# CoderWZW/ARLib

Measured on AMD Instinct MI355X. Metric: BPR-train interactions/sec (LightGCN d=64 L=3 + BPR + Adam, B=2048), higher is better.
Workload: dtype f32

## Files before the change

arlib_amd/_lib.py:

```python
import ctypes as C
import os

_HERE = os.path.dirname(os.path.abspath(__file__))
LIB_PATH = os.environ.get('ARLIB_AMD_LIB') or os.path.join(_HERE, 'lib', 'libarlib_amd.so')
ABI_VERSION = 34
_lib = None


class ArlError(RuntimeError):
    pass


class arl_csr(C.Structure):
    _fields_ = [('n_rows', C.c_int64), ('nnz', C.c_int64), ('rowptr', C.c_void_p), ('col', C.c_void_p), ('val', C.c_void_p),
                ('chunk', C.c_int32), ('n_chunks', C.c_int64), ('chunk_row', C.c_void_p), ('chunk_begin', C.c_void_p),
                ('chunk_end', C.c_void_p), ('n_long', C.c_int64), ('long_row', C.c_void_p), ('long_first', C.c_void_p),
                ('long_count', C.c_void_p), ('partial', C.c_void_p), ('row_tasks', C.c_void_p)]


class arl_blocked(C.Structure):
    _fields_ = [('n_waves', C.c_int64), ('rows_per_wave', C.c_int64), ('loads_in_flight', C.c_int64), ('wave_ptr', C.c_void_p), ('wave_rows', C.c_void_p), ('rec_col', C.c_void_p),
                ('rec_val', C.c_void_p), ('n_split', C.c_int64), ('split_row', C.c_void_p), ('split_first', C.c_void_p), ('split_count', C.c_void_p),
                ('partial', C.c_void_p), ('waves_per_group', C.c_int64)]

# ... 17 lines not shown
    'arl_spmm_blocked_flagged_f32': (C.c_int, [C.POINTER(arl_blocked), _vp, _i64, _vp, _f, _f, _vp, _vp, _vp, _vp]),
    'arl_spmm_csr_rscale_f32': (C.c_int, [C.POINTER(arl_csr), _vp, _i64, _vp, _f, _f, _vp, _vp, _vp]),
    'arl_spmm_blocked_rscale_f32': (C.c_int, [C.POINTER(arl_blocked), _vp, _i64, _vp, _f, _f, _vp, _vp, _vp]),
    'arl_spmm_blocked_layersum_f32': (C.c_int, [C.POINTER(arl_blocked), _vp, _i64, _vp, _vp, _vp, _vp]),
    'arl_spmm_blocked_adam_f32': (C.c_int, [C.POINTER(arl_blocked), _vp, _i64, _f, _f, _vp, _vp, _vp, _vp, _vp, _f, _f, _f, _f, _i64, _vp]),
    'arl_lpt_deal': (C.c_int, [_i64, _vp, _i64, _i64, _vp, _vp]),
    'arl_syn_v1_pairs': (_i64, [_i64, _i64, C.c_double, C.c_uint64, C.c_double, _i64, _i64, _vp, _i64]),
    'arl_graph_digest': (C.c_uint64, [_vp, _i64]),
    'arl_spmm_csr_flagged_f32': (C.c_int, [C.POINTER(arl_csr), _vp, _i64, _vp, _f, _f, _vp, _vp, _vp, _vp]),
    'arl_spmm_csr_rows_workspace_bytes': (_i64, [_i64, _i64, _i64]),
    'arl_spmm_csr_rows_f32': (C.c_int, [C.POINTER(arl_csr), _vp, _i64, _vp, _i64, _i64, _vp, _i64, _f, _vp, _vp, _vp, _vp]),
    'arl_spmm_csr_rows_pieces_f32': (C.c_int, [C.POINTER(arl_csr), _vp, _i64, _vp, _i64, _i64, _i64, _vp, _i64, _f, _vp, _vp, _vp, _vp]),
    'arl_spmm_csr_rows_scratch_offset': (_i64, [_i64, _i64, _i64]),
    'arl_mark_rows_u8': (C.c_int, [_vp, _vp, _i64, _i32, _vp]),
    'arl_mark_rows_bits_u32': (C.c_int, [_vp, _vp, _i64, _i32, _vp]),
    'arl_zero_rows_f32': (C.c_int, [_vp, _vp, _i64, _i64, _vp]),
    'arl_batch_rows_set_f32': (C.c_int, [_vp, _vp, _vp, _vp, _i64, _i64, _vp, _f, _vp, _vp, _vp]),
    'arl_batch_rows_clear_f32': (C.c_int, [_vp, _vp, _vp, _vp, _i64, _i64, _vp, _vp]),
    'arl_bpr_l2_workspace_bytes': (_i64, [_i64]),
    'arl_bpr_l2_fwd_bwd_f32': (C.c_int, [_vp, _i64, _i64, _vp, _vp, _vp, _i64, _f, _f, _vp, _vp, _vp, _i32, _vp]),
    'arl_bpr_l2_partial_f32': (C.c_int, [_vp, _i64, _i64, _vp, _vp, _vp, _i64, _i64, _vp, _vp, _vp]),
    'arl_bpr_l2_backward_f32': (C.c_int, [_vp, _i64, _i64, _vp, _vp, _vp, _i64, _f, _f, _vp, _vp, _vp, _vp]),
    'arl_adam_dense_f32': (C.c_int, [_vp, _vp, _vp, _vp, _i64, _f, _f, _f, _f, _i64, _vp]),
    'arl_sgd_dense_f32': (C.c_int, [_vp, _vp, _i64, _f, _vp]),
    'arl_gather_rows_f32': (C.c_int, [_vp, _vp, _i64, _i64, _vp, _vp]),
    'arl_scatter_add_rows_f32': (C.c_int, [_vp, _vp, _i64, _i64, _vp, _f, _vp]),
    'arl_rows_axpy_unique_f32': (C.c_int, [_vp, _vp, _vp, _i64, _i64, _f, _vp, _vp]),
    'arl_shard_batch_prep_i32': (C.c_int, [_vp, _vp, _vp, _i64, _i64, _i64, _vp, _vp, _vp, _vp, _vp]),
    'arl_infonce_workspace_bytes': (_i64, [_i64, _i64]),
    'arl_infonce_fwd_bwd_f32': (C.c_int, [_vp, _vp, _i64, _i64, _f, _f, _vp, _vp, _vp, _vp, _vp]),
    'arl_simgcl_perturb_f32': (C.c_int, [_vp, _vp, _i64, _i64, _f, _vp]),
    'arl_simgcl_perturb_rng_f32': (C.c_int, [_vp, _vp, _i64, _i64, _vp, _f, C.c_uint64, C.c_uint64, _vp]),
    'arl_ngcf_combine_f32': (C.c_int, [_vp, _vp, _i64, _i64, _vp, _vp]),
    'arl_ngcf_act_f32': (C.c_int, [_vp, _vp, _i64, _i64, _f, _vp]),
    'arl_ngcf_act_bwd_f32': (C.c_int, [_vp, _vp, _i64, _i64, _f, _vp, _vp]),
    'arl_ngcf_combine_bwd_f32': (C.c_int, [_vp, _vp, _vp, _i64, _i64, _vp, _vp, _vp]),
    'arl_ngcf_dense_fwd_f32': (C.c_int, [_vp, _vp, _vp, _i64, _i64, _f, _vp, _vp]),
    'arl_ngcf_dense_dgrad_f32': (C.c_int, [_vp, _vp, _vp, _vp, _vp, _i64, _i64, _f, _vp, _vp, _vp, _vp]),
    'arl_ngcf_wgrad_workspace_bytes': (_i64, [_i64, _i64]),
    'arl_ngcf_dense_wgrad_f32': (C.c_int, [_vp, _vp, _vp, _i64, _i64, _vp, _vp, _vp]),
    'arl_ncf_tower_fwd_f32': (C.c_int, [_vp, _vp, _vp, _i64, _i64, _vp, _vp, _vp, _vp, _vp, _vp, _vp, _vp, _vp, _vp]),
    'arl_ncf_tower_bwd_workspace_bytes': (_i64, [_i64, _i64]),
    'arl_ncf_tower_bwd_f32': (C.c_int, [_vp, _vp, _vp, _vp, _vp, _vp, _i64, _i64, _vp, _vp, _vp, _vp, _vp, _vp, _vp]),
    'arl_wrmf_l2_workspace_bytes': (_i64, [_i64]),
    'arl_wrmf_l2_fwd_bwd_f32': (C.c_int, [_vp, _i64, _i64, _vp, _vp, _vp, _i64, _f, _f, _f, _vp, _vp, _vp, _i32, _vp]),
    'arl_bpr_adv_workspace_bytes': (_i64, [_i64, _i64]),
    'arl_bpr_adv_fwd_bwd_f32': (C.c_int, [_vp, _i64, _i64, _vp, _vp, _vp, _i64, _vp, _f, _f, _vp, _vp, _vp, _vp, _i32, _vp]),
    'arl_sfa_workspace_bytes': (_i64, [_i64, _i64]),
    'arl_sfa_l1_fwd_bwd_f32': (C.c_int, [_vp, _vp, _vp, _i64, _i64, _i64, _f, C.c_int32, _vp, _vp, _vp, _vp]),
    'arl_sfa_stage1_f32': (C.c_int, [_vp, _vp, _vp, _i64, _i64, _vp, _vp, _vp]),
# ... 105 lines not shown
```

arlib_amd/csrc/arl_kernels.hip:

```cpp
#include <hip/hip_runtime.h>
#include <stdint.h>
#include <math.h>
#include <stdio.h>
#include "arlib_amd.h"
#include "arl_ordered.h"
#include <type_traits>

#define ARL_LAUNCH_CHECK()                                  \
    do {                                                    \
        hipError_t e__ = hipGetLastError();                 \
        if (e__ != hipSuccess) return (int)e__;             \
    } while (0)

namespace {

constexpr int kWave = 64;
constexpr int kBlock = 256;
constexpr int kWavesPerBlock = kBlock / kWave;

__device__ __forceinline__ float wave_sum(float v) {
#pragma unroll
    for (int off = 32; off > 0; off >>= 1) v += __shfl_xor(v, off);
    return v;
}
// ... 957 lines not shown
}

__global__ __launch_bounds__(kBlock) void rows_axpy_unique_kernel(float *__restrict__ dst, const float *__restrict__ src, const int32_t *__restrict__ idx,
                                                                   int c0, int c1, int d, float alpha, const uint32_t *__restrict__ dup, int lds_n) {
    extern __shared__ int32_t srows[];
    const int lane = threadIdx.x & 63;
    const int t = c0 + blockIdx.x * kWavesPerBlock + (threadIdx.x >> 6);
    const bool valid = t < c1;
    const long long row = valid ? idx[t] : 0;
    const bool scan = valid && (!dup || ((dup[row >> 5] >> (row & 31)) & 1u));
    if (lds_n > 0) {
        if (__syncthreads_or(scan)) stage_rows(srows, 0, lds_n, [&](int j) { return idx[j]; });
        if (!valid) return;
        if (scan && !ordered_scan_lds(srows, 0, t, t, (int)row, lane, [&](int) {})) return;
    } else {
        if (!valid) return;
        if (scan && !ordered_scan(0, t, t, row, lane, [&](int j) { return idx[j]; }, [&](int) {})) return;
    }
    float *o = dst + (size_t)row * d;
    const float *x = src + (size_t)row * d;
    for (int k = lane; k < d; k += kWave) o[k] = fmaf(alpha, x[k], o[k]);
}

__global__ __launch_bounds__(kBlock) void shard_batch_prep_kernel(const int32_t *__restrict__ u, const int32_t *__restrict__ p, const int32_t *__restrict__ n,
                                                                   int B, int u0, int u1, int32_t *__restrict__ lu, float *__restrict__ own,
                                                                   int32_t *__restrict__ item_rows, int32_t *__restrict__ rows_l) {
    const int b = blockIdx.x * kBlock + threadIdx.x;
    if (b >= B) return;
    const int Ul = u1 - u0;
    const int uu = u[b];
    const int l = min(max(uu - u0, 0), max(Ul - 1, 0));
    lu[b] = l; own[b] = (uu >= u0 && uu < u1) ? 1.f : 0.f; own[B + b] = 1.f; own[2 * B + b] = 1.f;
    const int pp = p[b], nn = n[b];
    item_rows[b] = pp; item_rows[B + b] = nn;
    rows_l[b] = l; rows_l[B + b] = Ul + pp; rows_l[2 * B + b] = Ul + nn;
}

__global__ __launch_bounds__(kBlock) void bpr_bwd_kernel(const float *__restrict__ emb, int d, long long item_off,
                                                          const int32_t *__restrict__ ui, const int32_t *__restrict__ pi,
                                                          const int32_t *__restrict__ ni, int B, float reg, float upstream,
                                                          const float *__restrict__ ws, const float *__restrict__ out,
                                                          float *__restrict__ G, int c0, int c1, int distinct) {
    extern __shared__ int32_t srows[];
    const int lane = threadIdx.x & 63;
    const int t = c0 + blockIdx.x * kWavesPerBlock + (threadIdx.x >> 6);
#define ARL_ROWOF_BPR(j) ((j) < B ? (long long)ui[j] : ((j) < 2 * B ? item_off + pi[(j) - B] : item_off + ni[(j) - 2 * B]))
    if (!distinct) stage_rows(srows, c0, c1, [&](int j) { return ARL_ROWOF_BPR(j); });
    if (t >= c1) return;
    const int row = (int)ARL_ROWOF_BPR(t);
    const float cu = out[2] > 0.f ? upstream * reg / out[2] : 0.f, cp = out[3] > 0.f ? upstream * reg / out[3] : 0.f;
    float *o = G + (size_t)row * d;
    const float *own = emb + (size_t)row * d;
    for (int k0 = 0; k0 < d; k0 += 256) {
        float acc[4], mine[4];
#pragma unroll
        for (int i = 0; i < 4; ++i) { const int k = k0 + 64 * i + lane; acc[i] = k < d ? o[k] : 0.f; mine[i] = k < d ? own[k] : 0.f; }
        auto term = [&](int tt) {
            const int kind = tt / B, b = tt - kind * B;
            const float g = ws[b] * upstream;
            const float *x = emb + (size_t)(kind == 0 ? item_off + pi[b] : (long long)ui[b]) * d;
            const float *y = emb + (size_t)(item_off + ni[b]) * d;
#pragma unroll
            for (int i = 0; i < 4; ++i) {
                const int k = k0 + 64 * i + lane;
                if (k < d) {
                    float c;
                    if (kind == 0) c = fmaf(g, x[k] - y[k], cu * mine[i]);
                    else if (kind == 1) c = fmaf(g, x[k], cp * mine[i]);
                    else c = -g * x[k];
                    acc[i] = __fadd_rn(acc[i], c);
                }
            }
        };
        if (distinct) term(t);
        else if (!ordered_scan_lds(srows, c0, c1, t, row, lane, term)) return;
#pragma unroll
        for (int i = 0; i < 4; ++i) { const int k = k0 + 64 * i + lane; if (k < d) o[k] = acc[i]; }
    }
#undef ARL_ROWOF_BPR
}

__global__ __launch_bounds__(kBlock) void adam_kernel(float4 *__restrict__ p, const float4 *__restrict__ g, float4 *__restrict__ m,
                                                       float4 *__restrict__ v, long long n4, float step_size, float bc2_sqrt,
                                                       float w1, float b2, float w2, float eps) {
    for (long long i = (long long)blockIdx.x * kBlock + threadIdx.x; i < n4; i += (long long)gridDim.x * kBlock) {
        const float4 g4 = g[i];
        float4 p4 = p[i], m4 = m[i], v4 = v[i];
        float gg[4] = {g4.x, g4.y, g4.z, g4.w}, pp[4] = {p4.x, p4.y, p4.z, p4.w}, mm[4] = {m4.x, m4.y, m4.z, m4.w}, vv[4] = {v4.x, v4.y, v4.z, v4.w};
#pragma unroll
        for (int k = 0; k < 4; ++k) {
            mm[k] = mm[k] + (gg[k] - mm[k]) * w1;
            vv[k] = vv[k] * b2 + w2 * gg[k] * gg[k];
            pp[k] = pp[k] - step_size * (mm[k] / (sqrtf(vv[k]) / bc2_sqrt + eps));
        }
        p[i] = make_float4(pp[0], pp[1], pp[2], pp[3]); m[i] = make_float4(mm[0], mm[1], mm[2], mm[3]); v[i] = make_float4(vv[0], vv[1], vv[2], vv[3]);
    }
}
__global__ __launch_bounds__(kBlock) void adam_scalar_kernel(float *p, const float *g, float *m, float *v, long long from, long long n,
                                                              float step_size, float bc2_sqrt, float w1, float b2, float w2, float eps) {
    for (long long i = from + (long long)blockIdx.x * kBlock + threadIdx.x; i < n; i += (long long)gridDim.x * kBlock) {
        const float gi = g[i];
        const float mi = m[i] + (gi - m[i]) * w1;
        const float vi = v[i] * b2 + w2 * gi * gi;
        m[i] = mi; v[i] = vi;
        p[i] = p[i] - step_size * (mi / (sqrtf(vi) / bc2_sqrt + eps));
    }
}
__global__ __launch_bounds__(kBlock) void sgd_kernel(float *__restrict__ p, const float *__restrict__ g, long long n, float lr) {
    for (long long i = (long long)blockIdx.x * kBlock + threadIdx.x; i < n; i += (long long)gridDim.x * kBlock) p[i] = p[i] - lr * g[i];
}

// ... 2931 lines not shown
    if (!dst || !idx) return ARL_E_NULL;
    if (n < 0 || d <= 0 || n > 0x7fffffffll || d > 0x7fffffffll) return ARL_E_ARG;
    if (n == 0) return ARL_OK;
    hipLaunchKernelGGL(zero_rows_kernel, dim3((unsigned)((n + kWavesPerBlock - 1) / kWavesPerBlock)), dim3(kBlock), 0, (hipStream_t)stream, dst, idx, (int)n, (int)d);
    ARL_LAUNCH_CHECK();
    return ARL_OK;
}

int64_t arl_bpr_l2_workspace_bytes(int64_t B) { return B < 0 ? 0 : (int64_t)sizeof(float) * 4 * B; }

int arl_bpr_l2_fwd_bwd_f32(const float *emb, int64_t d, int64_t item_off, const int32_t *u, const int32_t *p, const int32_t *n, int64_t B,
                           float reg, float upstream, float *loss_out, float *G, void *workspace, int32_t distinct_rows, arl_stream_t stream) {
    if (!emb || !u || !p || !n || !loss_out || !workspace) return ARL_E_NULL;
    if (d <= 0 || B <= 0 || item_off < 0) return ARL_E_ARG;
    if (B > 0x7fffffffll / 4 || d > 0x7fffffffll) return ARL_E_RANGE;
    hipStream_t st = (hipStream_t)stream;
    float *ws = (float *)workspace;
    const unsigned grid = (unsigned)((B + kWavesPerBlock - 1) / kWavesPerBlock);
    hipLaunchKernelGGL(bpr_fwd_kernel, dim3(grid), dim3(kBlock), 0, st, emb, (int)d, (long long)item_off, u, p, n, (int)B, (float)B, ws);
    ARL_LAUNCH_CHECK();
    hipLaunchKernelGGL(bpr_finalize_kernel, dim3(1), dim3(kBlock), 0, st, (int)B, reg, ws, loss_out, 0);
    ARL_LAUNCH_CHECK();
    if (G) {
        const int rc = launch_bpr_bwd(emb, d, item_off, u, p, n, B, reg, upstream, ws, loss_out, G, st, distinct_rows != 0);
        if (rc) return rc;
    }
    return ARL_OK;
}

int arl_bpr_l2_partial_f32(const float *emb, int64_t d, int64_t item_off, const int32_t *u, const int32_t *p, const int32_t *n, int64_t B_local,
                           int64_t B_global, float *sums_out, void *workspace, arl_stream_t stream) {
    if (!emb || !sums_out || !workspace) return ARL_E_NULL;
    if (B_local > 0 && (!u || !p || !n)) return ARL_E_NULL;
    if (d <= 0 || B_local < 0 || B_global < B_local || B_global <= 0 || item_off < 0) return ARL_E_ARG;
    if (B_local > 0x7fffffffll / 4 || d > 0x7fffffffll) return ARL_E_RANGE;
    hipStream_t st = (hipStream_t)stream;
    float *ws = (float *)workspace;
    if (B_local > 0) {
        const unsigned grid = (unsigned)((B_local + kWavesPerBlock - 1) / kWavesPerBlock);
        hipLaunchKernelGGL(bpr_fwd_kernel, dim3(grid), dim3(kBlock), 0, st, emb, (int)d, (long long)item_off, u, p, n, (int)B_local, (float)B_global, ws);
        ARL_LAUNCH_CHECK();
    }
    hipLaunchKernelGGL(bpr_finalize_kernel, dim3(1), dim3(kBlock), 0, st, (int)B_local, 0.f, ws, sums_out, 1);
    ARL_LAUNCH_CHECK();
    return ARL_OK;
}

int arl_bpr_l2_backward_f32(const float *emb, int64_t d, int64_t item_off, const int32_t *u, const int32_t *p, const int32_t *n, int64_t B_local,
                            float reg, float upstream, const float *norms4, float *G, const void *workspace, arl_stream_t stream) {
    if (!emb || !norms4 || !G || !workspace) return ARL_E_NULL;
    if (B_local > 0 && (!u || !p || !n)) return ARL_E_NULL;
    if (d <= 0 || B_local < 0 || item_off < 0) return ARL_E_ARG;
    if (B_local > 0x7fffffffll / 4 || d > 0x7fffffffll) return ARL_E_RANGE;
    if (B_local == 0) return ARL_OK;
    return launch_bpr_bwd(emb, d, item_off, u, p, n, B_local, reg, upstream, (const float *)workspace, norms4, G, (hipStream_t)stream);
}

int arl_adam_dense_f32(float *p, const float *g, float *m, float *v, int64_t n, float lr, float beta1, float beta2, float eps, int64_t step,
                       arl_stream_t stream) {
    if (!p || !g || !m || !v) return ARL_E_NULL;
    if (n < 0 || step < 1) return ARL_E_ARG;
    if (n == 0) return ARL_OK;
    const AdamScalars a = adam_scalars(lr, beta1, beta2, step);
    hipStream_t st = (hipStream_t)stream;
    const bool al = (((uintptr_t)p | (uintptr_t)g | (uintptr_t)m | (uintptr_t)v) & 15u) == 0;
    const long long n4 = al ? n / 4 : 0;
    if (n4 > 0) {
        hipLaunchKernelGGL(adam_kernel, dim3(grid_for(n4, kBlock)), dim3(kBlock), 0, st, (float4 *)p, (const float4 *)g, (float4 *)m, (float4 *)v, n4,
                           a.step_size, a.bc2_sqrt, a.w1, a.b2, a.w2, eps);
        ARL_LAUNCH_CHECK();
    }
    if (n4 * 4 < n) {
        hipLaunchKernelGGL(adam_scalar_kernel, dim3(grid_for(n - n4 * 4, kBlock)), dim3(kBlock), 0, st, p, g, m, v, n4 * 4, (long long)n, a.step_size,
                           a.bc2_sqrt, a.w1, a.b2, a.w2, eps);
        ARL_LAUNCH_CHECK();
    }
    return ARL_OK;
}

int arl_sgd_dense_f32(float *p, const float *g, int64_t n, float lr, arl_stream_t stream) {
    if (!p || !g) return ARL_E_NULL;
    if (n < 0) return ARL_E_ARG;
    if (n == 0) return ARL_OK;
    hipLaunchKernelGGL(sgd_kernel, dim3(grid_for(n, kBlock)), dim3(kBlock), 0, (hipStream_t)stream, p, g, (long long)n, lr);
    ARL_LAUNCH_CHECK();
    return ARL_OK;
}

int arl_tables_sum_f32(const float *const *tables, int64_t n_tables, int64_t n_elems, float alpha, float *out, arl_stream_t stream) {
    if (!tables || !out) return ARL_E_NULL;
    if (n_tables < 1 || n_tables > 8 || n_elems < 0 || (n_elems & 3)) return ARL_E_ARG;
    if (n_elems == 0) return ARL_OK;
// ... 21 lines not shown
    if (n < 0 || d <= 0 || n > 0x7fffffffll || d > 0x7fffffffll) return ARL_E_ARG;
    if (n == 0) return ARL_OK;
    for (int64_t c0 = 0; c0 < n; c0 += kOrderedWindow) {
        const int64_t c1 = c0 + kOrderedWindow < n ? c0 + kOrderedWindow : n;
        hipLaunchKernelGGL(rows_add_ordered_kernel<false>, dim3((unsigned)((c1 - c0 + kWavesPerBlock - 1) / kWavesPerBlock)), dim3(kBlock), (size_t)(c1 - c0) * 4,
                           (hipStream_t)stream, dst, (uint8_t *)nullptr, (uint32_t *)nullptr, idx, (int)c0, (int)c1, (int)d, src, scale, (const float *)nullptr,
                           (const uint32_t *)nullptr);
        ARL_LAUNCH_CHECK();
    }
    return ARL_OK;
}

int arl_rows_axpy_unique_f32(float *dst, const float *src, const int32_t *idx, int64_t n, int64_t d, float alpha, const uint32_t *dup_bits,
                             arl_stream_t stream) {
    if (!src || !idx || !dst) return ARL_E_NULL;
    if (n < 0 || d <= 0 || n > 0x7fffffffll || d > 0x7fffffffll || dst == src) return ARL_E_ARG;
    for (int64_t c0 = 0; c0 < n; c0 += kOrderedWindow) {
        const int64_t c1 = c0 + kOrderedWindow < n ? c0 + kOrderedWindow : n;
        const int lds_n = n <= kOrderedWindow ? (int)n : 0;
        hipLaunchKernelGGL(rows_axpy_unique_kernel, dim3((unsigned)((c1 - c0 + kWavesPerBlock - 1) / kWavesPerBlock)), dim3(kBlock), (size_t)lds_n * 4,
                           (hipStream_t)stream, dst, src, idx, (int)c0, (int)c1, (int)d, alpha, dup_bits, lds_n);
        ARL_LAUNCH_CHECK();
    }
    return ARL_OK;
}

int arl_shard_batch_prep_i32(const int32_t *u, const int32_t *p, const int32_t *n, int64_t B, int64_t u0, int64_t u1, int32_t *lu, float *own,
                             int32_t *item_rows, int32_t *rows_l, arl_stream_t stream) {
    if (!u || !p || !n || !lu || !own || !item_rows || !rows_l) return ARL_E_NULL;
    if (B < 0 || B > 0x7fffffffll / 3 || u0 < 0 || u1 < u0 || u1 > 0x7fffffffll) return ARL_E_ARG;
    if (B == 0) return ARL_OK;
    hipLaunchKernelGGL(shard_batch_prep_kernel, dim3((unsigned)((B + kBlock - 1) / kBlock)), dim3(kBlock), 0, (hipStream_t)stream, u, p, n, (int)B, (int)u0,
                       (int)u1, lu, own, item_rows, rows_l);
    ARL_LAUNCH_CHECK();
    return ARL_OK;
}

static int nce_allrows_splits(int64_t nA, int64_t nV) {
    const int64_t row_blocks = (nA + 63) / 64;
    int64_t s = (2048 + row_blocks - 1) / row_blocks;
    const int64_t max_s = (nV + 4095) / 4096;
    if (s > max_s) s = max_s;
    if (s > 512) s = 512;
    return (int)(s < 1 ? 1 : s);
}

// ... 855 lines not shown
```

arlib_amd/dist_engine.py:

```python
import ctypes as C
import os
from functools import partial

import numpy as np
import torch

from .attack._common import cw_term


class _TimedWork:

    def __init__(self, work, comm):
        self.work, self.comm = work, comm

    def wait(self):
        c = self.comm
        e0 = torch.cuda.Event(enable_timing=True); e1 = torch.cuda.Event(enable_timing=True)
        e0.record()
        self.work.wait()
        e1.record()
        c.waits.append((e0, e1))
        return True


# ... 378 lines not shown
        for h in range(L - 1):
            src, dst = layers[-1], self.hops[h]
            k.spmm(self.Ai, src, out=dst[Ul:])
            if pending is not None:
                pending.wait()
            pending = self.comm.all_reduce_async(dst[Ul:])
            k.spmm(self.Au, src, out=dst[:Ul])
            layers.append(dst)
        X = layers[-1]
        if pending is not None and L >= 2:
            mine = [t[Ul:] for j, t in enumerate(layers[:-1]) if j % self.world == self.rank]
        else:
            mine = [t[Ul:] for j, t in enumerate(layers) if j % self.world == self.rank]
        k.spmm_rows(self.Ai, X, item_rows, mine, s, out=self.C[B:], check_range=False)
        if pending is not None:
            pending.wait()
            if L >= 2 and (L - 1) % self.world == self.rank:
                self.C[B:].add_(k.gather_rows(X, item_rows_packed, check_range=False), alpha=s)
        if Ul:
            k.spmm_rows(self.Au, X, lu, [t[:Ul] for t in layers], s, out=self.C[:B], check_range=False, row_weight=own[:B])
        else:
            self.C[:B].zero_()
        self.comm.all_reduce(self.C)
        self.Gc.zero_()
        k.bpr_l2_fwd_bwd(self.C, B, self.ar, self.ar, self.arB, self.reg, self.Gc, workspace=self.ws, loss_out=self.loss_out, check_range=False, distinct_rows=True)
        k.batch_rows_set_(self.G, self.flags, self.bits, rows_l, self.Gc, 1.0, check_range=False, row_scale=own, dup_bits=self.dup_bits)
        self.t += 1
        zu = self.flags[:Ul]
        acc = self.G
        pending, prev_items, prev_a = None, None, 1.0
        for h in range(L):
            last = h == L - 1
            a = s if last else 1.0
            dst = self.hops[h % len(self.hops)]
            if dst is acc:
                dst = self.hops[(h + 1) % len(self.hops)]
            xf = self.bits if h == 0 else None
            k.spmm_flagged(self.Ai, acc, xf, a, 0.0, None, None, out=dst[Ul:])
            if pending is not None:
                pending.wait()
                k.rows_axpy_unique_(prev_items, self.G, item_rows_packed, prev_a, check_range=False, dup_bits=self.dup_bits)
            pending, prev_items, prev_a = self.comm.all_reduce_async(dst[Ul:]), dst, a
            if last:
                k.spmm_adam(self.Au, acc, a, a, self.G[:Ul], self.E0[:Ul], self.m[:Ul], self.v[:Ul], self.lr, self.t, self.betas, self.eps, zflags=zu)
            else:
                k.spmm_flagged(self.Au, acc, xf, a, a, self.G[:Ul], zu, out=dst[:Ul])
            acc = dst
        pending.wait()
        k.rows_axpy_unique_(prev_items, self.G, item_rows_packed, prev_a, check_range=False, dup_bits=self.dup_bits)
        k.adam_dense(self.E0[Ul:], acc[Ul:], self.m[Ul:], self.v[Ul:], self.lr, self.t, self.betas, self.eps)
        k.batch_rows_clear_(self.G, self.flags, self.bits, rows_l, check_range=False, dup_bits=self.dup_bits)
        return self.loss_out

    def step_simgcl(self, u, p, n, cl_rate=0.2, tau=0.2, eps=0.1, noises=None):
        if not self.skip0:
            raise ValueError('step_simgcl needs skip_layer0=True (SimGCL averages layers 1..L)')
        k, L, Ul, d, dev = self.k, self.L, self.Ul, self.d, self.device
        if self.S1 is None:
            self.S1, self.S2 = torch.zeros_like(self.S), torch.zeros_like(self.S)

        def noise(view, hop):
            if noises is not None:
                return noises[view][hop]
            g = torch.Generator(device=dev)
            g.manual_seed(0x51AC1 + 7919 * self.t + 2 * hop + view)
            item = torch.rand(self.I, d, generator=g, device=dev)
            return torch.cat([torch.rand(Ul, d, device=dev), item], 0)

        def perturb(view, h, dst):
            if noises is None and hasattr(k, 'simgcl_perturb_rng'):
                if self._gid is None:
                    self._gid = torch.cat([torch.arange(self.u0, self.u1, device=dev), torch.arange(self.U, self.U + self.I, device=dev)]).to(torch.int32)
                k.simgcl_perturb_rng(dst, eps, 0x51AC1, (self.t * 2 + view) * L + h, out=dst, row_ids=self._gid)
# ... 164 lines not shown
```

arlib_amd/engine.py:

```python
import torch

from . import ops


def mean_adjacency_gradient(A, E0, G, L, s, out, noises=None, eps=0.1):
    if L == 0:
        return out
    E = [E0]
    for k in range(L - 1):
        nxt = ops.spmm(A, E[-1])
        if noises is not None:
            ops.simgcl_perturb_(nxt, noises[k], eps)
        E.append(nxt)
    G = G.contiguous()
    acc = G
    for j in range(L):
        ops.sddmm_csr(A, acc, E[L - 1 - j], s, out=out)
        if j < L - 1:
            acc = ops.spmm(A, acc, 1.0, 1.0, G)
    return out


class PropagationEngine:
    def __init__(self, graph, n_users, n_items, emb_size, n_layers, reg, lr, device, skip_layer0=False,
# ... 130 lines not shown
    def _batch_rows(self, u, p, n):
        return torch.cat([u, p + self.U, n + self.U])

    def _contrast_rows(self, u, p):
        uidx = torch.unique(u.long())
        iidx = torch.unique(p.long()) + self.U
        return torch.cat([uidx, iidx]).to(torch.int32), uidx.numel()

    def _streams(self, n):
        if self._noise_seed is None:
            self._noise_seed = int(torch.randint(0, 2 ** 62, (1,)).item())
            self._noise_stream = 0
        first = self._noise_stream
        self._noise_stream += n
        return self._noise_seed, first

    def _mean_rows(self, graph, hops, rows, out=None, workspace=None):
        layers = [self.E0]
        for k in range(self.L - 1):
            layers.append(ops.spmm(graph, layers[-1], out=hops[k]))
        return ops.spmm_rows(graph, layers[-1], rows, layers, 1.0 / (self.L + 1), nsplit=self.nsplit, out=out, workspace=workspace, check_range=False)

    def _bpr_compact(self, out_c, B):
        self.Gc.zero_()
        ops.bpr_l2_fwd_bwd(out_c, B, self.ar, self.ar, self.arB, self.reg, self.Gc, workspace=self._ws, loss_out=self.loss_out, check_range=False, distinct_rows=True)

    def _set_rows(self, rows, grad):
        ops.batch_rows_set_(self.G, self.flags, self.bits, rows, grad, 1.0, check_range=False, dup_bits=self.dup_bits)

    def _mark_rows(self, rows):
        ops.mark_rows_(self.flags, rows, 1, check_range=False)
        ops.mark_bits_(self.bits, rows, True, self.N, check_range=False)

    def _clear_rows(self, rows):
        ops.batch_rows_clear_(self.G, self.flags, self.bits, rows, check_range=False, dup_bits=self.dup_bits)

    def _masked_hops(self, graph, bufs, src=None, after_hop=None):
        acc, bits = self.G if src is None else src, self.bits
        for k in range(self.L - 1):
            acc = ops.spmm_flagged(graph, acc, bits, 1.0, 1.0, self.G, self.flags, out=bufs[k % len(bufs)])
            bits = None
            if after_hop is not None:
                after_hop(self.L - 1 - k, acc)
        return acc, bits

    def loss_and_grad_out(self, out, u, p, n):
        self.G.zero_()
        self._G_dirty = True
# ... 348 lines not shown
```

arlib_amd/ops.py:

```python
import ctypes as C
import numpy as np
import torch

from . import _lib
from ._lib import arl_csr, check

DEFAULT_CHUNK = 512
EVENT_HOOK = None


_raw_stream = getattr(torch._C, '_cuda_getCurrentRawStream', None)


def _stream():
    if _raw_stream is not None:
        return C.c_void_p(_raw_stream(torch.cuda.current_device()))
    return C.c_void_p(torch.cuda.current_stream().cuda_stream)


def _dev(t, dtype, name, ndim=None):
    if not isinstance(t, torch.Tensor):
        raise TypeError('%s: expected a torch.Tensor' % name)
    if not t.is_cuda:
        raise _lib.ArlError('%s: must live on the GPU (no CPU fallback in arlib_amd)' % name)
# ... 699 lines not shown
def mark_bits_(bits, idx, set_, n_nodes, check_range=True):
    _dev(bits, torch.int32, 'bits', 1); _dev(idx, torch.int32, 'idx', 1)
    if bits.numel() != (n_nodes + 31) // 32:
        raise ValueError('mark_bits_: bitmap size')
    _check_rows(idx, n_nodes, 'mark_bits_', check_range)
    check(_lib.lib().arl_mark_rows_bits_u32(_ptr(bits), _ptr(idx), idx.numel(), 1 if set_ else 0, _stream()), 'arl_mark_rows_bits_u32')
    return bits


def zero_rows_(dst, idx, check_range=True):
    _dev(dst, torch.float32, 'dst', 2); _dev(idx, torch.int32, 'idx', 1)
    _check_rows(idx, dst.shape[0], 'zero_rows_', check_range)
    check(_lib.lib().arl_zero_rows_f32(_ptr(dst), _ptr(idx), idx.numel(), dst.shape[1], _stream()), 'arl_zero_rows_f32')
    return dst


def _check_idx(t, name, hi, B=None):
    _dev(t, torch.int32, name, 1)
    if B is not None and t.numel() != B:
        raise ValueError('%s: length %d != %d' % (name, t.numel(), B))
    return t


def bpr_l2_fwd_bwd(emb, item_off, u, p, n, reg, G=None, upstream=1.0, workspace=None, loss_out=None, check_range=True, distinct_rows=False):
    _dev(emb, torch.float32, 'emb', 2)
    N, d = emb.shape
    B = u.numel()
    for t, nm in ((u, 'u'), (p, 'p'), (n, 'n')):
        _check_idx(t, nm, N, B)
    if B == 0:
        raise ValueError('bpr_l2: empty batch')
    if check_range:
        mx = torch.stack([u.max(), p.max(), n.max(), -u.min(), -p.min(), -n.min()]).tolist()
        if mx[0] >= N or max(mx[1], mx[2]) + item_off >= N or max(mx[3:]) > 0:
            raise IndexError('bpr_l2: batch index out of range')
    if G is not None:
        _dev(G, torch.float32, 'G', 2)
        if G.shape != emb.shape:
            raise ValueError('bpr_l2: G shape mismatch')
    need = _lib.lib().arl_bpr_l2_workspace_bytes(B)
    if workspace is None or workspace.numel() * workspace.element_size() < need:
        workspace = torch.empty(need // 4, dtype=torch.float32, device=emb.device)
    if loss_out is None:
        loss_out = torch.empty(4, dtype=torch.float32, device=emb.device)
    check(_lib.lib().arl_bpr_l2_fwd_bwd_f32(_ptr(emb), d, item_off, _ptr(u), _ptr(p), _ptr(n), B, reg, upstream, _ptr(loss_out), _ptr(G),
                                            _ptr(workspace), 1 if distinct_rows else 0, _stream()), 'arl_bpr_l2_fwd_bwd_f32')
    return loss_out


def adam_dense(p, g, m, v, lr, step, betas=(0.9, 0.999), eps=1e-8):
    for t, nm in ((p, 'p'), (g, 'g'), (m, 'm'), (v, 'v')):
        _dev(t, torch.float32, nm)
        if t.numel() != p.numel():
            raise ValueError('adam_dense: size mismatch on %s' % nm)
    check(_lib.lib().arl_adam_dense_f32(_ptr(p), _ptr(g), _ptr(m), _ptr(v), p.numel(), lr, betas[0], betas[1], eps, int(step), _stream()), 'arl_adam_dense_f32')


def sgd_dense(p, g, lr):
    _dev(p, torch.float32, 'p'); _dev(g, torch.float32, 'g')
    if g.numel() != p.numel():
        raise ValueError('sgd_dense: size mismatch')
    check(_lib.lib().arl_sgd_dense_f32(_ptr(p), _ptr(g), p.numel(), lr, _stream()), 'arl_sgd_dense_f32')


def gather_rows(src, idx, check_range=True):
    _dev(src, torch.float32, 'src', 2); _dev(idx, torch.int32, 'idx', 1)
    _check_rows(idx, src.shape[0], 'gather_rows', check_range)
    dst = torch.empty(idx.numel(), src.shape[1], dtype=torch.float32, device=src.device)
    check(_lib.lib().arl_gather_rows_f32(_ptr(src), _ptr(idx), idx.numel(), src.shape[1], _ptr(dst), _stream()), 'arl_gather_rows_f32')
    return dst


def scatter_add_rows(dst, idx, src, scale=1.0, check_range=True):
    _dev(dst, torch.float32, 'dst', 2); _dev(src, torch.float32, 'src', 2); _dev(idx, torch.int32, 'idx', 1)
    if src.shape != (idx.numel(), dst.shape[1]):
        raise ValueError('scatter_add_rows: shape mismatch')
    _check_rows(idx, dst.shape[0], 'scatter_add_rows', check_range)
    check(_lib.lib().arl_scatter_add_rows_f32(_ptr(dst), _ptr(idx), idx.numel(), dst.shape[1], _ptr(src), scale, _stream()), 'arl_scatter_add_rows_f32')
    return dst


def rows_axpy_unique_(dst, src, idx, alpha=1.0, check_range=True, dup_bits=None):
    _dev(dst, torch.float32, 'dst', 2); _dev(src, torch.float32, 'src', 2); _dev(idx, torch.int32, 'idx', 1)
    if src.shape != dst.shape or src.data_ptr() == dst.data_ptr():
        raise ValueError('rows_axpy_unique_: dst and src must be distinct tables of one shape')
    _check_rows(idx, dst.shape[0], 'rows_axpy_unique_', check_range)
    check(_lib.lib().arl_rows_axpy_unique_f32(_ptr(dst), _ptr(src), _ptr(idx), idx.numel(), dst.shape[1], float(alpha), _ptr(dup_bits), _stream()), 'arl_rows_axpy_unique_f32')
    return dst


def shard_batch_prep(u, p, n, u0, u1, out=None):
    for t, nm in ((u, 'u'), (p, 'p'), (n, 'n')):
        _dev(t, torch.int32, nm, 1)
    B = u.numel()
    if p.numel() != B or n.numel() != B or not (0 <= u0 <= u1):
        raise ValueError('shard_batch_prep: u, p, n must have one length and 0 <= u0 <= u1')
    if out is None:
        out = (torch.empty(B, dtype=torch.int32, device=u.device), torch.empty(3 * B, dtype=torch.float32, device=u.device),
               torch.empty(2 * B, dtype=torch.int32, device=u.device), torch.empty(3 * B, dtype=torch.int32, device=u.device))
    lu, own, item_rows, rows_l = out
    check(_lib.lib().arl_shard_batch_prep_i32(_ptr(u), _ptr(p), _ptr(n), B, int(u0), int(u1), _ptr(lu), _ptr(own), _ptr(item_rows), _ptr(rows_l), _stream()),
          'arl_shard_batch_prep_i32')
    return out


def infonce_fwd_bwd(v1, v2, tau, want_grad=True, upstream=1.0):
    _dev(v1, torch.float32, 'v1', 2); _dev(v2, torch.float32, 'v2', 2)
    if v1.shape != v2.shape:
        raise ValueError('infonce: shape mismatch')
    n, d = v1.shape
# ... 891 lines not shown
```

include/arlib_amd.h:

```cpp
#ifndef ARLIB_AMD_H
#define ARLIB_AMD_H

#include <stdint.h>

#ifdef __cplusplus
extern "C" {
#endif

#define ARL_OK 0
#define ARL_E_NULL (-1)
#define ARL_E_DIM (-2)
#define ARL_E_RANGE (-3)
#define ARL_E_ARG (-4)

typedef void *arl_stream_t;

int arl_abi_version(void);

int arl_mt_seed(uint32_t *mt_state, const uint32_t *key, int64_t key_len);
int arl_sampler_shuffle(uint32_t *mt_state, int32_t *pairs, int64_t nnz);
int arl_mt_sample_range(uint32_t *mt_state, int64_t n, int64_t k, int32_t use_pool, int32_t *out, int32_t *scratch);
int64_t arl_goat_item_sample_scratch_words(int64_t n_items, int64_t k, int64_t n_targets);
int arl_goat_item_sample(uint32_t *mt_state, const int64_t *rowptr, const int32_t *items, int64_t n_users, int64_t n_items,
                         const double *int_num, const int32_t *targets, int64_t n_targets, int64_t n_fake, int64_t k, double min_items,
// ... 81 lines not shown
int arl_spmm_blocked_adam_f32(const arl_blocked *P, const float *X, int64_t d, float alpha, float beta, const float *Z,
                              const uint8_t *zflags, float *Pm, float *M, float *V, float lr, float beta1, float beta2,
                              float eps, int64_t step, arl_stream_t stream);
int arl_lpt_deal(int64_t n, const int32_t *weight_desc, int64_t n_bins, int64_t cap, int32_t *bin_out, int32_t *slot_out);

int64_t arl_syn_v1_pairs(int64_t n_users, int64_t n_items, double mean_deg, uint64_t seed, double sigma, int64_t deg_min, int64_t deg_max,
                         int32_t *pairs_out, int64_t capacity);
uint64_t arl_graph_digest(const int32_t *pairs, int64_t n);

int64_t arl_bpr_l2_workspace_bytes(int64_t B);
int arl_bpr_l2_fwd_bwd_f32(const float *emb, int64_t d, int64_t item_off, const int32_t *u, const int32_t *p,
                           const int32_t *n, int64_t B, float reg, float upstream, float *loss_out, float *G,
                           void *workspace, int32_t distinct_rows, arl_stream_t stream);

int arl_bpr_l2_partial_f32(const float *emb, int64_t d, int64_t item_off, const int32_t *u, const int32_t *p,
                           const int32_t *n, int64_t B_local, int64_t B_global, float *sums_out, void *workspace,
                           arl_stream_t stream);
int arl_bpr_l2_backward_f32(const float *emb, int64_t d, int64_t item_off, const int32_t *u, const int32_t *p,
                            const int32_t *n, int64_t B_local, float reg, float upstream, const float *norms4, float *G,
                            const void *workspace, arl_stream_t stream);

int arl_adam_dense_f32(float *p, const float *g, float *m, float *v, int64_t n, float lr, float beta1,
                       float beta2, float eps, int64_t step, arl_stream_t stream);
int arl_sgd_dense_f32(float *p, const float *g, int64_t n, float lr, arl_stream_t stream);

int arl_gather_rows_f32(const float *src, const int32_t *idx, int64_t n, int64_t d, float *dst, arl_stream_t stream);
int arl_scatter_add_rows_f32(float *dst, const int32_t *idx, int64_t n, int64_t d, const float *src, float scale,
                             arl_stream_t stream);
int arl_rows_axpy_unique_f32(float *dst, const float *src, const int32_t *idx, int64_t n, int64_t d, float alpha,
                             const uint32_t *dup_bits, arl_stream_t stream);
int arl_shard_batch_prep_i32(const int32_t *u, const int32_t *p, const int32_t *n, int64_t B, int64_t u0, int64_t u1,
                             int32_t *lu, float *own, int32_t *item_rows, int32_t *rows_l, arl_stream_t stream);

int64_t arl_infonce_workspace_bytes(int64_t n, int64_t d);
int arl_infonce_fwd_bwd_f32(const float *v1, const float *v2, int64_t n, int64_t d, float tau, float upstream,
                            float *loss_out, float *dv1, float *dv2, void *workspace, arl_stream_t stream);

int arl_simgcl_perturb_f32(float *E, const float *noise, int64_t n, int64_t d, float eps, arl_stream_t stream);
int arl_simgcl_perturb_rng_f32(const float *src, float *dst, int64_t n, int64_t d, const int32_t *row_ids, float eps, uint64_t seed,
                               uint64_t stream_id, arl_stream_t stream);

int arl_ngcf_combine_f32(const float *P, const float *E, int64_t n, int64_t d, float *ST, arl_stream_t stream);
int arl_ngcf_act_f32(float *Z, float *acc, int64_t n, int64_t d, float slope, arl_stream_t stream);
int arl_ngcf_act_bwd_f32(const float *gOut, const float *Out, int64_t n, int64_t d, float slope, float *gZ, arl_stream_t stream);
int arl_ngcf_combine_bwd_f32(const float *gST, const float *P, const float *E, int64_t n, int64_t d, float *gP, float *gE,
                             arl_stream_t stream);
int arl_ngcf_dense_fwd_f32(const float *P, const float *E, const float *W, int64_t n, int64_t d, float slope, float *out, arl_stream_t stream);
int arl_ngcf_dense_dgrad_f32(const float *gOut, const float *Out, const float *P, const float *E, const float *Wt, int64_t n, int64_t d, float slope,
                             float *gZ, float *gP, float *gE, arl_stream_t stream);
int64_t arl_ngcf_wgrad_workspace_bytes(int64_t n, int64_t d);
int arl_ngcf_dense_wgrad_f32(const float *P, const float *E, const float *gZ, int64_t n, int64_t d, float *gW, void *workspace, arl_stream_t stream);

int arl_ncf_tower_fwd_f32(const float *mf, const float *mlp, const int32_t *rows, int64_t n, int64_t d, const float *W0, const float *b0,
// ... 165 lines not shown
```

Before: 331,900.

## Fuse item-row axpy into Adam and let BPR overwrite its gradient buffer

New measurement: 331,800. No clear change (-0.0%).

```diff
diff --git a/arlib_amd/_lib.py b/arlib_amd/_lib.py
--- a/arlib_amd/_lib.py
+++ b/arlib_amd/_lib.py
@@ -63,10 +63,12 @@
     'arl_bpr_l2_partial_f32': (C.c_int, [_vp, _i64, _i64, _vp, _vp, _vp, _i64, _i64, _vp, _vp, _vp]),
     'arl_bpr_l2_backward_f32': (C.c_int, [_vp, _i64, _i64, _vp, _vp, _vp, _i64, _f, _f, _vp, _vp, _vp, _vp]),
     'arl_adam_dense_f32': (C.c_int, [_vp, _vp, _vp, _vp, _i64, _f, _f, _f, _f, _i64, _vp]),
+    'arl_adam_dense_rows_f32': (C.c_int, [_vp, _vp, _vp, _vp, _i64, _i64, _f, _vp, _vp, _f, _f, _f, _f, _i64, _vp]),
     'arl_sgd_dense_f32': (C.c_int, [_vp, _vp, _i64, _f, _vp]),
     'arl_gather_rows_f32': (C.c_int, [_vp, _vp, _i64, _i64, _vp, _vp]),
     'arl_scatter_add_rows_f32': (C.c_int, [_vp, _vp, _i64, _i64, _vp, _f, _vp]),
     'arl_rows_axpy_unique_f32': (C.c_int, [_vp, _vp, _vp, _i64, _i64, _f, _vp, _vp]),
+    'arl_rows_axpy_flagged_f32': (C.c_int, [_vp, _vp, _vp, _i64, _i64, _f, _vp]),
     'arl_shard_batch_prep_i32': (C.c_int, [_vp, _vp, _vp, _i64, _i64, _i64, _vp, _vp, _vp, _vp, _vp]),
     'arl_infonce_workspace_bytes': (_i64, [_i64, _i64]),
     'arl_infonce_fwd_bwd_f32': (C.c_int, [_vp, _vp, _i64, _i64, _f, _f, _vp, _vp, _vp, _vp, _vp]),
diff --git a/arlib_amd/csrc/arl_kernels.hip b/arlib_amd/csrc/arl_kernels.hip
--- a/arlib_amd/csrc/arl_kernels.hip
+++ b/arlib_amd/csrc/arl_kernels.hip
@@ -1003,6 +1003,21 @@
     for (int k = lane; k < d; k += kWave) o[k] = fmaf(alpha, x[k], o[k]);
 }
 
+__global__ __launch_bounds__(kBlock) void rows_axpy_flagged_kernel(float *__restrict__ dst, const float *__restrict__ src, const uint8_t *__restrict__ flags,
+                                                                    int n_rows, int d, float alpha) {
+    const int lane = threadIdx.x & 63;
+    const long long r0 = ((long long)blockIdx.x * kWavesPerBlock + (threadIdx.x >> 6)) * kWave;
+    if (r0 >= n_rows) return;
+    unsigned long long todo = __ballot(r0 + lane < n_rows && flags[r0 + lane] != 0);
+    while (todo) {
+        const long long row = r0 + __builtin_ctzll(todo);
+        todo &= todo - 1ull;
+        float *o = dst + (size_t)row * d;
+        const float *x = src + (size_t)row * d;
+        for (int k = lane; k < d; k += kWave) o[k] = fmaf(alpha, x[k], o[k]);
+    }
+}
+
 __global__ __launch_bounds__(kBlock) void shard_batch_prep_kernel(const int32_t *__restrict__ u, const int32_t *__restrict__ p, const int32_t *__restrict__ n,
                                                                    int B, int u0, int u1, int32_t *__restrict__ lu, float *__restrict__ own,
                                                                    int32_t *__restrict__ item_rows, int32_t *__restrict__ rows_l) {
@@ -1035,7 +1050,7 @@
     for (int k0 = 0; k0 < d; k0 += 256) {
         float acc[4], mine[4];
 #pragma unroll
-        for (int i = 0; i < 4; ++i) { const int k = k0 + 64 * i + lane; acc[i] = k < d ? o[k] : 0.f; mine[i] = k < d ? own[k] : 0.f; }
+        for (int i = 0; i < 4; ++i) { const int k = k0 + 64 * i + lane; acc[i] = (k < d && distinct != 2) ? o[k] : 0.f; mine[i] = k < d ? own[k] : 0.f; }
         auto term = [&](int tt) {
             const int kind = tt / B, b = tt - kind * B;
             const float g = ws[b] * upstream;
@@ -1061,13 +1076,24 @@
 #undef ARL_ROWOF_BPR
 }
 
+struct AdamZ {
+    const float *Z; const uint8_t *zflags; float beta; int d, d4, sh;
+};
+template <bool ZROWS>
 __global__ __launch_bounds__(kBlock) void adam_kernel(float4 *__restrict__ p, const float4 *__restrict__ g, float4 *__restrict__ m,
                                                        float4 *__restrict__ v, long long n4, float step_size, float bc2_sqrt,
-                                                       float w1, float b2, float w2, float eps) {
+                                                       float w1, float b2, float w2, float eps, AdamZ z) {
     for (long long i = (long long)blockIdx.x * kBlock + threadIdx.x; i < n4; i += (long long)gridDim.x * kBlock) {
         const float4 g4 = g[i];
         float4 p4 = p[i], m4 = m[i], v4 = v[i];
         float gg[4] = {g4.x, g4.y, g4.z, g4.w}, pp[4] = {p4.x, p4.y, p4.z, p4.w}, mm[4] = {m4.x, m4.y, m4.z, m4.w}, vv[4] = {v4.x, v4.y, v4.z, v4.w};
+        if constexpr (ZROWS) {
+            const long long row = z.sh >= 0 ? i >> z.sh : i / z.d4;
+            if (!z.zflags || z.zflags[row]) {
+                const float4 z4 = reinterpret_cast<const float4 *>(z.Z)[i];
+                gg[0] = fmaf(z.beta, z4.x, gg[0]); gg[1] = fmaf(z.beta, z4.y, gg[1]); gg[2] = fmaf(z.beta, z4.z, gg[2]); gg[3] = fmaf(z.beta, z4.w, gg[3]);
+            }
+        }
 #pragma unroll
         for (int k = 0; k < 4; ++k) {
             mm[k] = mm[k] + (gg[k] - mm[k]) * w1;
@@ -4045,7 +4071,7 @@
     hipLaunchKernelGGL(bpr_finalize_kernel, dim3(1), dim3(kBlock), 0, st, (int)B, reg, ws, loss_out, 0);
     ARL_LAUNCH_CHECK();
     if (G) {
-        const int rc = launch_bpr_bwd(emb, d, item_off, u, p, n, B, reg, upstream, ws, loss_out, G, st, distinct_rows != 0);
+        const int rc = launch_bpr_bwd(emb, d, item_off, u, p, n, B, reg, upstream, ws, loss_out, G, st, distinct_rows == 2 ? 2 : distinct_rows != 0);
         if (rc) return rc;
     }
     return ARL_OK;
@@ -4079,6 +4105,23 @@
     return launch_bpr_bwd(emb, d, item_off, u, p, n, B_local, reg, upstream, (const float *)workspace, norms4, G, (hipStream_t)stream);
 }
 
+int arl_adam_dense_rows_f32(float *p, const float *g, float *m, float *v, int64_t n_rows, int64_t d, float beta, const float *Z, const uint8_t *zflags,
+                            float lr, float beta1, float beta2, float eps, int64_t step, arl_stream_t stream) {
+    if (!p || !g || !m || !v || !Z) return ARL_E_NULL;
+    if (n_rows < 0 || d < 4 || (d & 3) || step < 1) return ARL_E_ARG;
+    if (d > 0x7fffffffll || n_rows > 0x7fffffffll) return ARL_E_RANGE;
+    if ((((uintptr_t)p | (uintptr_t)g | (uintptr_t)m | (uintptr_t)v | (uintptr_t)Z) & 15u) != 0) return ARL_E_ARG;
+    if (n_rows == 0) return ARL_OK;
+    const AdamScalars a = adam_scalars(lr, beta1, beta2, step);
+    const int d4 = (int)(d / 4);
+    const AdamZ z = {Z, zflags, beta, (int)d, d4, (d4 & (d4 - 1)) == 0 ? __builtin_ctz((unsigned)d4) : -1};
+    const long long n4 = (long long)n_rows * d4;
+    hipLaunchKernelGGL(adam_kernel<true>, dim3(grid_for(n4, kBlock)), dim3(kBlock), 0, (hipStream_t)stream, (float4 *)p, (const float4 *)g, (float4 *)m,
+                       (float4 *)v, n4, a.step_size, a.bc2_sqrt, a.w1, a.b2, a.w2, eps, z);
+    ARL_LAUNCH_CHECK();
+    return ARL_OK;
+}
+
 int arl_adam_dense_f32(float *p, const float *g, float *m, float *v, int64_t n, float lr, float beta1, float beta2, float eps, int64_t step,
                        arl_stream_t stream) {
     if (!p || !g || !m || !v) return ARL_E_NULL;
@@ -4089,8 +4132,8 @@
     const bool al = (((uintptr_t)p | (uintptr_t)g | (uintptr_t)m | (uintptr_t)v) & 15u) == 0;
     const long long n4 = al ? n / 4 : 0;
     if (n4 > 0) {
-        hipLaunchKernelGGL(adam_kernel, dim3(grid_for(n4, kBlock)), dim3(kBlock), 0, st, (float4 *)p, (const float4 *)g, (float4 *)m, (float4 *)v, n4,
-                           a.step_size, a.bc2_sqrt, a.w1, a.b2, a.w2, eps);
+        hipLaunchKernelGGL(adam_kernel<false>, dim3(grid_for(n4, kBlock)), dim3(kBlock), 0, st, (float4 *)p, (const float4 *)g, (float4 *)m, (float4 *)v, n4,
+                           a.step_size, a.bc2_sqrt, a.w1, a.b2, a.w2, eps, AdamZ{});
         ARL_LAUNCH_CHECK();
     }
     if (n4 * 4 < n) {
@@ -4158,6 +4201,17 @@
                            (hipStream_t)stream, dst, src, idx, (int)c0, (int)c1, (int)d, alpha, dup_bits, lds_n);
         ARL_LAUNCH_CHECK();
     }
+    return ARL_OK;
+}
+
+int arl_rows_axpy_flagged_f32(float *dst, const float *src, const uint8_t *flags, int64_t n_rows, int64_t d, float alpha, arl_stream_t stream) {
+    if (!src || !flags || !dst) return ARL_E_NULL;
+    if (n_rows < 0 || d <= 0 || n_rows > 0x7fffffffll || d > 0x7fffffffll || dst == src) return ARL_E_ARG;
+    if (n_rows == 0) return ARL_OK;
+    const int64_t per_block = (int64_t)kWavesPerBlock * kWave;
+    hipLaunchKernelGGL(rows_axpy_flagged_kernel, dim3((unsigned)((n_rows + per_block - 1) / per_block)), dim3(kBlock), 0, (hipStream_t)stream, dst, src, flags,
+                       (int)n_rows, (int)d, alpha);
+    ARL_LAUNCH_CHECK();
     return ARL_OK;
 }
 
diff --git a/arlib_amd/dist_engine.py b/arlib_amd/dist_engine.py
--- a/arlib_amd/dist_engine.py
+++ b/arlib_amd/dist_engine.py
@@ -424,8 +424,12 @@
         else:
             self.C[:B].zero_()
         self.comm.all_reduce(self.C)
-        self.Gc.zero_()
-        k.bpr_l2_fwd_bwd(self.C, B, self.ar, self.ar, self.arB, self.reg, self.Gc, workspace=self.ws, loss_out=self.loss_out, check_range=False, distinct_rows=True)
+        if getattr(k, 'BPR_OVERWRITE', False):
+            k.bpr_l2_fwd_bwd(self.C, B, self.ar, self.ar, self.arB, self.reg, self.Gc, workspace=self.ws, loss_out=self.loss_out, check_range=False, distinct_rows=True,
+                             overwrite=True)
+        else:
+            self.Gc.zero_()
+            k.bpr_l2_fwd_bwd(self.C, B, self.ar, self.ar, self.arB, self.reg, self.Gc, workspace=self.ws, loss_out=self.loss_out, check_range=False, distinct_rows=True)
         k.batch_rows_set_(self.G, self.flags, self.bits, rows_l, self.Gc, 1.0, check_range=False, row_scale=own, dup_bits=self.dup_bits)
         self.t += 1
         zu = self.flags[:Ul]
@@ -441,7 +445,10 @@
             k.spmm_flagged(self.Ai, acc, xf, a, 0.0, None, None, out=dst[Ul:])
             if pending is not None:
                 pending.wait()
-                k.rows_axpy_unique_(prev_items, self.G, item_rows_packed, prev_a, check_range=False, dup_bits=self.dup_bits)
+                if hasattr(k, 'rows_axpy_flagged_'):
+                    k.rows_axpy_flagged_(prev_items[Ul:], self.G[Ul:], self.flags[Ul:], prev_a)
+                else:
+                    k.rows_axpy_unique_(prev_items, self.G, item_rows_packed, prev_a, check_range=False, dup_bits=self.dup_bits)
             pending, prev_items, prev_a = self.comm.all_reduce_async(dst[Ul:]), dst, a
             if last:
                 k.spmm_adam(self.Au, acc, a, a, self.G[:Ul], self.E0[:Ul], self.m[:Ul], self.v[:Ul], self.lr, self.t, self.betas, self.eps, zflags=zu)
@@ -449,8 +456,11 @@
                 k.spmm_flagged(self.Au, acc, xf, a, a, self.G[:Ul], zu, out=dst[:Ul])
             acc = dst
         pending.wait()
-        k.rows_axpy_unique_(prev_items, self.G, item_rows_packed, prev_a, check_range=False, dup_bits=self.dup_bits)
-        k.adam_dense(self.E0[Ul:], acc[Ul:], self.m[Ul:], self.v[Ul:], self.lr, self.t, self.betas, self.eps)
+        if getattr(k, 'ADAM_DENSE_ROWS', False):
+            k.adam_dense(self.E0[Ul:], acc[Ul:], self.m[Ul:], self.v[Ul:], self.lr, self.t, self.betas, self.eps, Z=self.G[Ul:], zflags=self.flags[Ul:], beta=prev_a)
+        else:
+            k.rows_axpy_unique_(prev_items, self.G, item_rows_packed, prev_a, check_range=False, dup_bits=self.dup_bits)
+            k.adam_dense(self.E0[Ul:], acc[Ul:], self.m[Ul:], self.v[Ul:], self.lr, self.t, self.betas, self.eps)
         k.batch_rows_clear_(self.G, self.flags, self.bits, rows_l, check_range=False, dup_bits=self.dup_bits)
         return self.loss_out
 
diff --git a/arlib_amd/engine.py b/arlib_amd/engine.py
--- a/arlib_amd/engine.py
+++ b/arlib_amd/engine.py
@@ -176,8 +176,8 @@
         return ops.spmm_rows(graph, layers[-1], rows, layers, 1.0 / (self.L + 1), nsplit=self.nsplit, out=out, workspace=workspace, check_range=False)
 
     def _bpr_compact(self, out_c, B):
-        self.Gc.zero_()
-        ops.bpr_l2_fwd_bwd(out_c, B, self.ar, self.ar, self.arB, self.reg, self.Gc, workspace=self._ws, loss_out=self.loss_out, check_range=False, distinct_rows=True)
+        ops.bpr_l2_fwd_bwd(out_c, B, self.ar, self.ar, self.arB, self.reg, self.Gc, workspace=self._ws, loss_out=self.loss_out, check_range=False, distinct_rows=True,
+                           overwrite=True)
 
     def _set_rows(self, rows, grad):
         ops.batch_rows_set_(self.G, self.flags, self.bits, rows, grad, 1.0, check_range=False, dup_bits=self.dup_bits)
diff --git a/arlib_amd/ops.py b/arlib_amd/ops.py
--- a/arlib_amd/ops.py
+++ b/arlib_amd/ops.py
@@ -745,7 +745,9 @@
     return t
 
 
-def bpr_l2_fwd_bwd(emb, item_off, u, p, n, reg, G=None, upstream=1.0, workspace=None, loss_out=None, check_range=True, distinct_rows=False):
+def bpr_l2_fwd_bwd(emb, item_off, u, p, n, reg, G=None, upstream=1.0, workspace=None, loss_out=None, check_range=True, distinct_rows=False, overwrite=False):
+    if overwrite and not distinct_rows:
+        raise ValueError('bpr_l2: overwrite needs distinct_rows')
     _dev(emb, torch.float32, 'emb', 2)
     N, d = emb.shape
     B = u.numel()
@@ -767,15 +769,32 @@
     if loss_out is None:
         loss_out = torch.empty(4, dtype=torch.float32, device=emb.device)
     check(_lib.lib().arl_bpr_l2_fwd_bwd_f32(_ptr(emb), d, item_off, _ptr(u), _ptr(p), _ptr(n), B, reg, upstream, _ptr(loss_out), _ptr(G),
-                                            _ptr(workspace), 1 if distinct_rows else 0, _stream()), 'arl_bpr_l2_fwd_bwd_f32')
+                                            _ptr(workspace), (2 if overwrite else 1) if distinct_rows else 0, _stream()), 'arl_bpr_l2_fwd_bwd_f32')
     return loss_out
 
 
-def adam_dense(p, g, m, v, lr, step, betas=(0.9, 0.999), eps=1e-8):
+BPR_OVERWRITE = True
+ADAM_DENSE_ROWS = True
+
+
+def adam_dense(p, g, m, v, lr, step, betas=(0.9, 0.999), eps=1e-8, Z=None, zflags=None, beta=0.0):
     for t, nm in ((p, 'p'), (g, 'g'), (m, 'm'), (v, 'v')):
         _dev(t, torch.float32, nm)
         if t.numel() != p.numel():
             raise ValueError('adam_dense: size mismatch on %s' % nm)
+    if Z is not None:
+        _dev(Z, torch.float32, 'Z', 2)
+        if p.dim() != 2 or Z.shape != p.shape or Z.shape[1] % 4:
+            raise ValueError('adam_dense: Z needs p as a [n, d] table of its shape, d a multiple of 4')
+        if zflags is not None and _dev(zflags, torch.uint8, 'zflags', 1).numel() != p.shape[0]:
+            raise ValueError('adam_dense: zflags must have one byte per row')
+        if any(Z.data_ptr() == t.data_ptr() for t in (p, m, v)):
+            raise ValueError('adam_dense: Z must not alias p, m or v')
+        check(_lib.lib().arl_adam_dense_rows_f32(_ptr(p), _ptr(g), _ptr(m), _ptr(v), p.shape[0], p.shape[1], float(beta), _ptr(Z), _ptr(zflags), lr,
+                                                 betas[0], betas[1], eps, int(step), _stream()), 'arl_adam_dense_rows_f32')
+        return
+    if zflags is not None:
+        raise ValueError('adam_dense: zflags without Z')
     check(_lib.lib().arl_adam_dense_f32(_ptr(p), _ptr(g), _ptr(m), _ptr(v), p.numel(), lr, betas[0], betas[1], eps, int(step), _stream()), 'arl_adam_dense_f32')
 
 
@@ -809,6 +828,14 @@
         raise ValueError('rows_axpy_unique_: dst and src must be distinct tables of one shape')
     _check_rows(idx, dst.shape[0], 'rows_axpy_unique_', check_range)
     check(_lib.lib().arl_rows_axpy_unique_f32(_ptr(dst), _ptr(src), _ptr(idx), idx.numel(), dst.shape[1], float(alpha), _ptr(dup_bits), _stream()), 'arl_rows_axpy_unique_f32')
+    return dst
+
+
+def rows_axpy_flagged_(dst, src, flags, alpha=1.0):
+    _dev(dst, torch.float32, 'dst', 2); _dev(src, torch.float32, 'src', 2); _dev(flags, torch.uint8, 'flags', 1)
+    if src.shape != dst.shape or src.data_ptr() == dst.data_ptr() or flags.numel() != dst.shape[0]:
+        raise ValueError('rows_axpy_flagged_: dst and src must be distinct tables of one shape, flags one byte per row')
+    check(_lib.lib().arl_rows_axpy_flagged_f32(_ptr(dst), _ptr(src), _ptr(flags), dst.shape[0], dst.shape[1], float(alpha), _stream()), 'arl_rows_axpy_flagged_f32')
     return dst
 
 
diff --git a/include/arlib_amd.h b/include/arlib_amd.h
--- a/include/arlib_amd.h
+++ b/include/arlib_amd.h
@@ -127,6 +127,8 @@
 
 int arl_adam_dense_f32(float *p, const float *g, float *m, float *v, int64_t n, float lr, float beta1,
                        float beta2, float eps, int64_t step, arl_stream_t stream);
+int arl_adam_dense_rows_f32(float *p, const float *g, float *m, float *v, int64_t n_rows, int64_t d, float beta, const float *Z,
+                            const uint8_t *zflags, float lr, float beta1, float beta2, float eps, int64_t step, arl_stream_t stream);
 int arl_sgd_dense_f32(float *p, const float *g, int64_t n, float lr, arl_stream_t stream);
 
 int arl_gather_rows_f32(const float *src, const int32_t *idx, int64_t n, int64_t d, float *dst, arl_stream_t stream);
@@ -134,6 +136,7 @@
                              arl_stream_t stream);
 int arl_rows_axpy_unique_f32(float *dst, const float *src, const int32_t *idx, int64_t n, int64_t d, float alpha,
                              const uint32_t *dup_bits, arl_stream_t stream);
+int arl_rows_axpy_flagged_f32(float *dst, const float *src, const uint8_t *flags, int64_t n_rows, int64_t d, float alpha, arl_stream_t stream);
 int arl_shard_batch_prep_i32(const int32_t *u, const int32_t *p, const int32_t *n, int64_t B, int64_t u0, int64_t u1,
                              int32_t *lu, float *own, int32_t *item_rows, int32_t *rows_l, arl_stream_t stream);
 
```
